# ilya16/deephumor

Measured on AMD Instinct MI355X. Metric: captions/sec (224x224, 32-tok, beam=5), higher is better.
Workload: dtype bf16; 1 GPU; C2 CaptioningLSTM + ImageEncoder (emb 256, hidden 512, 2 layers); images_per_gpu=256, global_batch=256, vocab=36541, max_len=32, beam_size=5, top_k=50, parallelism=image-sharded x1, one all_gather of token ids per batch, weights=synthetic name-keyed (seed 1234), inputs=device-resident fp32 NCHW images (host-inclusive rates under host_inclusive), hipgraph=False, schedule=sequential: one batch at a time

## Files before the change

deephumor_amd/csrc/beam.hip:

```cpp
#include "common.h"
#include "prof.h"

#define CAP DH_BEAM_MAX_SURVIVORS

__device__ __forceinline__ uint32_t f2key(float f) {
    uint32_t u = __float_as_uint(f);
    if (u == 0x80000000u) u = 0u;
    return (u & 0x80000000u) ? ~u : (u | 0x80000000u);
}


__device__ __forceinline__ void radix_pick_digit(const int* hist, int n_hist, int shift, uint32_t prefix,
                                                 uint32_t* s_prefix, int* s_k, int* wtot) {
    const int tid = threadIdx.x, lane = tid & 63, wave = tid >> 6;
    const int k = *s_k;
    int c = 0, suf = 0;
    if (tid < 256) {
        for (int h = 0; h < n_hist; ++h) c += hist[h * 256 + tid];
        suf = c;
        suf += __builtin_amdgcn_update_dpp(0, suf, 0x101, 0xF, 0xF, true);
        suf += __builtin_amdgcn_update_dpp(0, suf, 0x102, 0xF, 0xF, true);
        suf += __builtin_amdgcn_update_dpp(0, suf, 0x104, 0xF, 0xF, true);
        suf += __builtin_amdgcn_update_dpp(0, suf, 0x108, 0xF, 0xF, true);
        {
// ... 726 lines not shown
#pragma unroll
            for (int k = 0; k < MB; ++k) if (k == b) { was = was_ended[k] != 0; vb = val_b[k]; if constexpr (LN) kb = key_b[k]; }
            const int tok = was ? 0 : (pre ? L.pki[b * B + j] : p.pick_idx[(size_t)(base + b) * B + j]);
            ctok[c] = tok;
            cval[c] = vb + (was ? 0.f : (pre ? L.pkv[b * B + j] : p.pick_val[(size_t)(base + b) * B + j]));
            if constexpr (LN) q[c] = was ? kb : cval[c] * w_len;
            cpar[c] = b;
            cend[c] = (uint8_t)(was || tok == p.eos);
        }
        if (lane == 0) s_n = total;
    }
    wave_lds_sync();
    const int n = s_n;
    if constexpr (PL) {
        beam_pool_tail<MB>(p, img, lane, L, n, first, pre);
        return;
    }
    if constexpr (GR) {
        beam_group_tail(p, lane, L, n, first);
    } else if constexpr (DT) {
        if (!first) {
            for (int j = lane; j < B; j += 64) keep[j] = min(j, n - 1);
            wave_lds_sync();
            const float* rank = LN ? q : cval;
            for (int c = lane; c < n; c += 64) {
                const float me = rank[c];
                int r = 0;
                for (int j = 0; j < n; ++j) r += (rank[j] > me) || (rank[j] == me && j < c);
                if (r < B) keep[r] = c;
            }
        }
    } else if (!first) {
        float m = -INFINITY;
        for (int c = lane; c < n; c += 64) m = fmaxf(m, cval[c] / p.temperature);
        m = wave_max(m);
        float s = 0.f;
        for (int c = lane; c < n; c += 64) { const float e = expf(cval[c] / p.temperature - m); q[c] = e; s += e; }
        s = wave_sum(s);
        for (int c = lane; c < n; c += 64) {
            const float nz = p.noise ? p.noise[(size_t)img * B * B + c]
                                     : philox_exp1(p.seed ^ (p.seed_ptr ? *p.seed_ptr : 0ull), (uint32_t)(p.img0 + img), (uint32_t)p.step_index, 1u, 0u, (uint32_t)c);
            q[c] = (q[c] / s) / nz;
        }
        for (int j = lane; j < B; j += 64) keep[j] = min(j, n - 1);
        wave_lds_sync();
        for (int c = lane; c < n; c += 64) {
            const float me = q[c];
            int r = 0;
            for (int j = 0; j < n; ++j) r += (q[j] > me) || (q[j] == me && j < c);
            if (r < B) keep[r] = c;
        }
    }
    int32_t* tokbuf = stage;
    int32_t* srcbuf = stage + (size_t)B * p.tok_ld;
    if (!pre) {
        for (int i = lane; i < B * p.tok_ld; i += 64) tokbuf[i] = p.tokens[(size_t)base * p.tok_ld + i];
        if (p.src)
            for (int b = 0; b < B; ++b)
                for (int j = lane; j < p.t; j += 64) srcbuf[b * p.t + j] = p.src[(size_t)(base + b) * p.src_ld + j];
    }
    wave_lds_sync();
    int all_ended = 1;
    for (int b = 0; b < B; ++b) {
        const int c = keep[b], par = cpar[c];
        for (int i = lane; i < p.tok_ld; i += 64)
            p.tokens[(size_t)(base + b) * p.tok_ld + i] = (i == p.write_pos) ? ctok[c] : tokbuf[par * p.tok_ld + i];
        if (p.src) {
            for (int j = lane; j < p.t; j += 64) p.src[(size_t)(base + b) * p.src_ld + j] = srcbuf[par * p.t + j];
            if (lane == 0) p.src[(size_t)(base + b) * p.src_ld + p.t] = base + par;
        }
        if (lane == 0) {
            p.vals[base + b] = cval[c];
            if constexpr (LN) p.keys[base + b] = q[c];
            p.ended[base + b] = cend[c];
            p.parent[base + b] = base + par;
            p.hparent[base + b] = DT ? base + par : base + c / B;
        }
        all_ended &= cend[c];
    }
    if (lane == 0 && all_ended && !first) { p.done[img] = 1; p.end_step[img] = p.step_index; }
#undef s_n
}

template <int NT, bool PR, bool NU = false>
__global__ __launch_bounds__(NT) void beam_row_sample_groups_kernel(
    const float* __restrict__ logits, int ldl, int V, const float* __restrict__ gmax, int gm_ld, int n_groups,
    int gcols, int rows_per_img, int beam, int top_k, float temperature, int unk, const float* __restrict__ noise,
    uint64_t seed, const uint64_t* __restrict__ seed_ptr, int img0, int step, int32_t* __restrict__ pick_idx, float* __restrict__ pick_val,
    int32_t* __restrict__ err, const int32_t* __restrict__ first_pos, float top_p) {
    constexpr int MAXG = 1024, GPT = MAXG / NT;
    __shared__ int glist[MAXG];
    __shared__ int hist[4][256];
    __shared__ uint32_t s_prefix, s_thr;
    __shared__ int s_k, s_cnt, s_ng, wtot[4];
    __shared__ __attribute__((aligned(16))) int32_t pool[5 * CAP];
    int* const idx_a = pool; int* const idx_b = pool + CAP;
    float* const val_a = reinterpret_cast<float*>(pool + 2 * CAP); float* const val_b = reinterpret_cast<float*>(pool + 3 * CAP);
    float* const qv = reinterpret_cast<float*>(pool + 4 * CAP);
    __shared__ float red[NT];
    __shared__ int picks[DH_BEAM_MAX_BEAMS];
    const int rc = blockIdx.x, tid = threadIdx.x, lane = tid & 63, wave = tid >> 6;
    if constexpr (PR) { if (prompt_row_idle(first_pos, rc, rows_per_img, step)) return; }
    const float* row = logits + (size_t)rc * ldl;
    uint32_t gk[GPT];
#pragma unroll
    for (int e = 0; e < GPT; ++e) {
        const int g = tid + e * NT;
        const uint32_t k = f2key(gmax[(size_t)rc * gm_ld + min(g, n_groups - 1)]);
        gk[e] = g < n_groups ? k : 0u;
    }
    for (int i = tid; i < 512; i += NT) (&hist[0][0])[i] = 0;
    if (tid == 0) { s_prefix = 0u; s_k = min(top_k, n_groups); s_cnt = 0; s_ng = 0; s_thr = 0u; }
    __syncthreads();
#pragma unroll
    for (int pass = 0; pass < 2; ++pass) {
        const int shift = 24 - 8 * pass;
        const uint32_t prefix = s_prefix, mask = pass == 0 ? 0u : 0xFF000000u;
#pragma unroll
        for (int e = 0; e < GPT; ++e)
            if (tid + e * NT < n_groups && (gk[e] & mask) == prefix) atomicAdd(&hist[pass][(gk[e] >> shift) & 255u], 1);
        __syncthreads();
        radix_pick_digit(hist[pass], 1, shift, prefix, &s_prefix, &s_k, wtot);
    }
    const uint32_t bound = s_prefix;
#pragma unroll
    for (int e = 0; e < GPT; ++e)
        if (tid + e * NT < n_groups && gk[e] >= bound) glist[atomicAdd(&s_ng, 1)] = tid + e * NT;
    __syncthreads();
    const int ng = s_ng;
    constexpr int NWV = NT / 64, UN = 16;
    for (int q0 = wave; q0 < ng; q0 += NWV * UN) {
        float v[UN]; int ci[UN];
#pragma unroll
        for (int u = 0; u < UN; ++u) {
            const int q = q0 + u * NWV;
            ci[u] = q < ng ? glist[min(q, ng - 1)] * gcols + lane : V;
            v[u] = row[min(ci[u], V - 1)];
        }
#pragma unroll
        for (int u = 0; u < UN; ++u)
            if (lane < gcols && ci[u] < V && f2key(v[u]) >= bound) {
                const int pp = atomicAdd(&s_cnt, 1);
                if (pp < CAP) { idx_a[pp] = ci[u]; val_a[pp] = v[u]; }
            }
    }
    __syncthreads();
    if (s_cnt > CAP) radix_row_candidates<NT>(row, V, top_k, &hist[0][0], &s_prefix, &s_k, &s_cnt, wtot, idx_a, val_a);
    const RowLds L{idx_a, idx_b, val_a, val_b, qv, red, picks, &s_cnt, &s_thr};
    row_tail<NT, NU>(L, rc, ldl, rows_per_img, beam, top_k, temperature, unk, noise, seed, seed_ptr, img0, step, pick_idx, pick_val, err, top_p);
}

template <bool PR, bool NU = false>
static int row_sample_groups_launch(const float* logits, int ldl, int V, const float* group_max, int gm_ld,
                                    int n_groups, int group_cols, int rows, int rows_per_img, int beam,
                                    int top_k, float temperature, int unk_index, const float* noise,
                                    uint64_t seed, const uint64_t* seed_ptr, int img0, int step, const int32_t* first_pos,
                                    int32_t* pick_idx, float* pick_val, int32_t* err, void* stream, float top_p = 1.f) {
    DH_REQUIRE(logits && group_max && pick_idx && pick_val && err && rows > 0 && rows_per_img > 0 && V > 0 && ldl >= V);
    DH_REQUIRE(beam >= 1 && beam <= DH_BEAM_MAX_BEAMS && beam <= top_k && top_k <= V && temperature > 0.f);
    DH_REQUIRE(n_groups > 0 && n_groups <= 1024 && top_k <= n_groups && gm_ld >= n_groups && group_cols > 0 && group_cols <= 64 &&
               (long long)n_groups * group_cols >= V);
    DH_REQUIRE(!PR || (first_pos && rows_per_img == beam && rows % beam == 0));
    DhProfScope prof(NU ? "dh_beam_row_sample_nucleus" : "dh_beam_row_sample", 0.0, 0.0, stream);
    hipLaunchKernelGGL((beam_row_sample_groups_kernel<256, PR, NU>), dim3(rows), dim3(256), 0, (hipStream_t)stream, logits, ldl, V,
                       group_max, gm_ld, n_groups, group_cols, rows_per_img, beam, top_k, temperature, unk_index, noise,
                       seed, seed_ptr, img0, step, pick_idx, pick_val, err, first_pos, top_p);
    DH_LAUNCH_CHECK();
}

extern "C" int dh_beam_row_sample_groups(const float* logits, int ldl, int V, const float* group_max, int gm_ld,
                                         int n_groups, int group_cols, int rows, int rows_per_img, int beam,
                                         int top_k, float temperature, int unk_index, const float* noise,
                                         uint64_t seed, const uint64_t* __restrict__ seed_ptr, int img0, int step, int32_t* pick_idx, float* pick_val,
                                         int32_t* err, void* stream) {
    return row_sample_groups_launch<false>(logits, ldl, V, group_max, gm_ld, n_groups, group_cols, rows, rows_per_img, beam, top_k, temperature,
                                           unk_index, noise, seed, seed_ptr, img0, step, nullptr, pick_idx, pick_val, err, stream);
}

extern "C" int dh_beam_row_sample_groups_prompted(const float* logits, int ldl, int V, const float* group_max, int gm_ld,
                                                  int n_groups, int group_cols, int rows, int rows_per_img, int beam,
                                                  int top_k, float temperature, int unk_index, const float* noise,
                                                  uint64_t seed, const uint64_t* seed_ptr, int img0, int step, const int32_t* first_pos,
                                                  int32_t* pick_idx, float* pick_val, int32_t* err, void* stream) {
    return row_sample_groups_launch<true>(logits, ldl, V, group_max, gm_ld, n_groups, group_cols, rows, rows_per_img, beam, top_k, temperature,
                                          unk_index, noise, seed, seed_ptr, img0, step, first_pos, pick_idx, pick_val, err, stream);
}

template <bool PR, bool NU = false>
static int row_sample_launch(const float* logits, int ldl, int V, int rows, int rows_per_img, int beam,
                             int top_k, float temperature, int unk_index, const float* noise,
                             uint64_t seed, const uint64_t* seed_ptr, int img0, int step, const int32_t* first_pos, int32_t* pick_idx,
                             float* pick_val, int32_t* err, bool exact, void* stream, float top_p = 1.f) {
    DH_REQUIRE(logits && pick_idx && pick_val && err && rows > 0 && rows_per_img > 0 && V > 0 && ldl >= V);
    DH_REQUIRE(beam >= 1 && beam <= DH_BEAM_MAX_BEAMS && beam <= top_k && top_k <= V && temperature > 0.f);
    DH_REQUIRE(!PR || (first_pos && rows_per_img == beam && rows % beam == 0));
    DhProfScope prof(NU ? "dh_beam_row_sample_nucleus" : "dh_beam_row_sample", 0.0, 0.0, stream);
#define DH_FAST(EPT, NT, WPE) hipLaunchKernelGGL((beam_row_sample_fast_kernel<EPT, NT, WPE, PR, NU>), dim3(rows), dim3(NT), 0, \
        (hipStream_t)stream, logits, ldl, V, rows_per_img, beam, top_k, temperature, unk_index, noise, seed, seed_ptr, img0, \
        step, pick_idx, pick_val, err, first_pos, top_p)
    if (!exact && top_k <= 256 && V <= 512 * 8) DH_FAST(8, 512, 4);
    else if (!exact && top_k <= 256 && V <= 1024 * 16) DH_FAST(16, 1024, 8);
    else if (!exact && top_k <= 256 && V <= 1024 * 36) DH_FAST(36, 1024, 8);
    else if (!exact && top_k <= 256 && V <= 1024 * 64) DH_FAST(64, 1024, 4);
    else
        hipLaunchKernelGGL((beam_row_sample_kernel<PR, NU>), dim3(rows), dim3(256), 0, (hipStream_t)stream, logits, ldl, V,
                           rows_per_img, beam, top_k, temperature, unk_index, noise, seed, seed_ptr, img0, step, pick_idx,
                           pick_val, err, first_pos, top_p);
#undef DH_FAST
    DH_LAUNCH_CHECK();
}

extern "C" int dh_beam_row_sample(const float* logits, int ldl, int V, int rows, int rows_per_img, int beam,
                                  int top_k, float temperature, int unk_index, const float* noise,
                                  uint64_t seed, const uint64_t* __restrict__ seed_ptr, int img0, int step, int32_t* pick_idx, float* pick_val,
                                  int32_t* err, void* stream) {
    return row_sample_launch<false>(logits, ldl, V, rows, rows_per_img, beam, top_k, temperature, unk_index, noise, seed, seed_ptr, img0, step,
                                    nullptr, pick_idx, pick_val, err, false, stream);
}

extern "C" int dh_beam_row_sample_exact(const float* logits, int ldl, int V, int rows, int rows_per_img, int beam,
                                        int top_k, float temperature, int unk_index, const float* noise,
                                        uint64_t seed, const uint64_t* __restrict__ seed_ptr, int img0, int step, int32_t* pick_idx, float* pick_val,
                                        int32_t* err, void* stream) {
    return row_sample_launch<false>(logits, ldl, V, rows, rows_per_img, beam, top_k, temperature, unk_index, noise, seed, seed_ptr, img0, step,
                                    nullptr, pick_idx, pick_val, err, true, stream);
}

extern "C" int dh_beam_row_sample_prompted(const float* logits, int ldl, int V, int rows, int rows_per_img, int beam,
                                           int top_k, float temperature, int unk_index, const float* noise,
                                           uint64_t seed, const uint64_t* seed_ptr, int img0, int step, const int32_t* first_pos,
                                           int32_t* pick_idx, float* pick_val, int32_t* err, void* stream) {
    return row_sample_launch<true>(logits, ldl, V, rows, rows_per_img, beam, top_k, temperature, unk_index, noise, seed, seed_ptr, img0, step,
                                   first_pos, pick_idx, pick_val, err, false, stream);
}

extern "C" int dh_beam_row_sample_exact_prompted(const float* logits, int ldl, int V, int rows, int rows_per_img, int beam,
                                                 int top_k, float temperature, int unk_index, const float* noise,
                                                 uint64_t seed, const uint64_t* seed_ptr, int img0, int step, const int32_t* first_pos,
                                                 int32_t* pick_idx, float* pick_val, int32_t* err, void* stream) {
    return row_sample_launch<true>(logits, ldl, V, rows, rows_per_img, beam, top_k, temperature, unk_index, noise, seed, seed_ptr, img0, step,
                                   first_pos, pick_idx, pick_val, err, true, stream);
}

extern "C" int dh_beam_row_sample_nucleus(const float* logits, int ldl, int V, const float* group_max, int gm_ld, int n_groups,
                                          int group_cols, int rows, int rows_per_img, int beam, int top_k, float top_p,
                                          float temperature, int unk_index, const float* noise, uint64_t seed, const uint64_t* seed_ptr,
                                          int img0, int step, const int32_t* first_pos, int exact, int32_t* pick_idx, float* pick_val,
                                          int32_t* err, void* stream) {
    DH_REQUIRE(top_p > 0.f && top_p < 1.f);
// ... 418 lines not shown
    p.diversity = diversity_penalty;
    const size_t lds = (size_t)beam * (tok_ld + (src ? t : 0)) * sizeof(int32_t);
    DH_REQUIRE(lds <= 56 * 1024);
    const dim3 grid(n_img), block(64);
    if (first_pos) {
        if (beam <= 16) hipLaunchKernelGGL((beam_select_groups_kernel<16, true>), grid, block, lds, (hipStream_t)stream, p);
        else hipLaunchKernelGGL((beam_select_groups_kernel<DH_BEAM_MAX_BEAMS, true>), grid, block, lds, (hipStream_t)stream, p);
    } else {
        if (beam <= 16) hipLaunchKernelGGL((beam_select_groups_kernel<16, false>), grid, block, lds, (hipStream_t)stream, p);
        else hipLaunchKernelGGL((beam_select_groups_kernel<DH_BEAM_MAX_BEAMS, false>), grid, block, lds, (hipStream_t)stream, p);
    }
    DH_LAUNCH_CHECK();
}

__global__ __launch_bounds__(64) void beam_finalize_pool_kernel(
    const int32_t* __restrict__ tokens, int tok_ld, const float* __restrict__ keys, const uint8_t* __restrict__ ended,
    const uint8_t* __restrict__ done, const int32_t* __restrict__ pool_tokens, const float* __restrict__ pool_keys,
    const int32_t* __restrict__ pool_len, const int32_t* __restrict__ pool_n, int32_t* __restrict__ out_tokens, int out_ld,
    int32_t* __restrict__ out_len, float* __restrict__ out_score, int32_t* __restrict__ out_index, int32_t* __restrict__ out_drawn,
    int32_t* __restrict__ out_row_len, int beam, int full_len, int pad_index) {
    __shared__ int s_from[DH_BEAM_MAX_BEAMS], s_len[DH_BEAM_MAX_BEAMS];
    const int img = blockIdx.x, lane = threadIdx.x, B = beam, base = img * B;
    const int cap = min(out_ld, tok_ld);
    const int n_pool = min(max(pool_n[img], 0), B);
    const bool in_pool = lane < n_pool;
    const bool live = lane < B && !done[img] && !ended[base + lane];
    float pk = in_pool ? pool_keys[base + lane] : -INFINITY;
    float lk = live ? keys[base + lane] : -INFINITY;
    if (!(pk == pk)) pk = -INFINITY;
    if (!(lk == lk)) lk = -INFINITY;
    const int plen = in_pool ? min(max(pool_len[base + lane], 0), cap) : 0;
    const int llen = min(max(full_len, 0), cap);
    int prank = lane, lrank = 0;
    for (int j = 0; j < B; ++j) {
        const float opk = __shfl(pk, j), olk = __shfl(lk, j);
        const bool o_pool = j < n_pool, o_live = __shfl((int)live, j) != 0;
        prank += o_live && olk > pk;
        lrank += (o_pool && opk >= lk) + (o_live && (olk > lk || (olk == lk && j < lane)));
    }
    const int n_live = __popcll(__ballot(live));
    const int total = n_pool + n_live;
    const unsigned long long idle = __ballot(lane < B && !live);
    const int frank = total + __popcll(idle & ((1ull << lane) - 1ull));
    if (lane < B) { s_from[lane] = lane; s_len[lane] = 0; }
    __syncthreads();
    if (in_pool && prank < B) {
        s_from[prank] = -1 - lane; s_len[prank] = plen;
        out_score[base + prank] = pk; out_index[base + prank] = -1; out_len[base + prank] = plen;
    }
    if (live && lrank < B) {
        s_from[lrank] = lane; s_len[lrank] = llen;
        out_score[base + lrank] = lk; out_index[base + lrank] = lane; out_len[base + lrank] = llen;
    }
    if (lane < B && !live && frank < B) {
        s_from[frank] = lane; s_len[frank] = llen;
        out_score[base + frank] = -INFINITY; out_index[base + frank] = lane; out_len[base + frank] = llen;
    }
    __syncthreads();
    if (lane == 0) { out_drawn[img] = 0; out_row_len[img] = s_len[0]; }
    for (int s = 0; s < B; ++s) {
        const int from = s_from[s], len = s_len[s];
        const int32_t* __restrict__ row = from < 0 ? pool_tokens + (size_t)(base + (-1 - from)) * tok_ld : tokens + (size_t)(base + from) * tok_ld;
        int32_t* __restrict__ dst = out_tokens + (size_t)(base + s) * out_ld;
        for (int i = lane; i < out_ld; i += 64) dst[i] = i < len ? row[i] : pad_index;
    }
}

extern "C" int dh_beam_finalize_pool(const int32_t* tokens, int tok_ld, const float* keys, const uint8_t* ended, const uint8_t* done,
                                     const int32_t* pool_tokens, const float* pool_keys, const int32_t* pool_len, const int32_t* pool_n,
                                     int32_t* out_tokens, int out_ld, int32_t* out_len, float* out_score, int32_t* out_index,
                                     int32_t* out_drawn, int32_t* out_row_len, int n_img, int beam, int full_len, int pad_index,
                                     void* stream) {
    DH_REQUIRE(tokens && keys && ended && done && pool_tokens && pool_keys && pool_len && pool_n);
    DH_REQUIRE(out_tokens && out_len && out_score && out_index && out_drawn && out_row_len);
    DH_REQUIRE(n_img > 0 && tok_ld > 0 && out_ld > 0 && full_len >= 0 && beam >= 1 && beam <= DH_BEAM_MAX_BEAMS);
    DhProfScope prof("dh_beam_finalize_pool", 0.0, 0.0, stream);
    hipLaunchKernelGGL(beam_finalize_pool_kernel, dim3(n_img), dim3(64), 0, (hipStream_t)stream, tokens, tok_ld, keys, ended, done,
                       pool_tokens, pool_keys, pool_len, pool_n, out_tokens, out_ld, out_len, out_score, out_index, out_drawn, out_row_len,
                       beam, full_len, pad_index);
    DH_LAUNCH_CHECK();
}


__device__ __forceinline__ float key2f(uint32_t k) {
    return __uint_as_float((k & 0x80000000u) ? (k & 0x7FFFFFFFu) : ~k);
}

__global__ __launch_bounds__(256) void beam_filter_topk_kernel(float* __restrict__ logits, int ldl, int V, int top_k, int unk) {
    __shared__ int hist[4 * 256];
    __shared__ uint32_t s_prefix;
    __shared__ int s_k, wtot[4];
    const int tid = threadIdx.x, hw = tid >> 6;
    float* row = logits + (size_t)blockIdx.x * ldl;
    if (tid == 0) { s_prefix = 0u; s_k = top_k; }
    uint32_t mask = 0u;
    for (int pass = 0; pass < 4; ++pass) {
        const int shift = 24 - 8 * pass;
        for (int i = tid; i < 1024; i += 256) hist[i] = 0;
        __syncthreads();
        const uint32_t prefix = s_prefix;
        for (int i = tid; i < V; i += 256) {
            const uint32_t key = f2key(row[i]);
            if ((key & mask) == prefix) atomicAdd(&hist[hw * 256 + ((key >> shift) & 255u)], 1);
        }
        __syncthreads();
        radix_pick_digit(hist, 4, shift, prefix, &s_prefix, &s_k, wtot);
        mask |= 0xFFu << shift;
    }
    const float thr = key2f(s_prefix);
    for (int i = tid; i < V; i += 256)
        if (row[i] < thr || i == unk) row[i] = -INFINITY;
}

__global__ __launch_bounds__(256) void beam_sample_k_kernel(const float* __restrict__ x, int ld, int V, int k, float temperature,
                                                            const float* __restrict__ noise, int noise_ld, uint64_t seed,
                                                            const uint64_t* __restrict__ seed_ptr, int stream_id, int draw,
                                                            int64_t* __restrict__ out, int32_t* __restrict__ err) {
    __shared__ float red[256];
    __shared__ float rq[256];
    __shared__ int ri[256];
    __shared__ int picked[64];
    const int tid = threadIdx.x, r = blockIdx.x;
    const float* row = x + (size_t)r * ld;
    float m = -INFINITY;
    for (int i = tid; i < V; i += 256) m = fmaxf(m, row[i] / temperature);
    m = block_reduce_256(m, red, true);
    if (m == -INFINITY) {
        if (tid == 0) atomicOr(err, DH_BEAM_ERR_ALL_FILTERED);
        for (int j = tid; j < k; j += 256) out[(size_t)r * k + j] = 0;
        return;
    }
    float s = 0.f, cnt = 0.f;
    for (int i = tid; i < V; i += 256) { const float e = expf(row[i] / temperature - m); s += e; cnt += e > 0.f ? 1.f : 0.f; }
    s = block_reduce_256(s, red, false);
    cnt = block_reduce_256(cnt, red, false);
    if (tid == 0 && cnt < (float)k) atomicOr(err, DH_BEAM_ERR_TOO_FEW);
    const uint64_t sd = seed ^ (seed_ptr ? *seed_ptr : 0ull);
    for (int round = 0; round < k; ++round) {
        float bq = -1.f; int bi = 0x7FFFFFFF;
        for (int i = tid; i < V; i += 256) {
            bool taken = false;
            for (int j = 0; j < round; ++j) taken |= picked[j] == i;
            if (taken) continue;
            const float nz = noise ? noise[(size_t)r * noise_ld + i] : philox_exp1(sd, (uint32_t)stream_id, (uint32_t)draw, 3u, (uint32_t)r, (uint32_t)i);
            const float q = (expf(row[i] / temperature - m) / s) / nz;
            if (q > bq) { bq = q; bi = i; }
        }
        rq[tid] = bq; ri[tid] = bi;
        __syncthreads();
        for (int st = 128; st > 0; st >>= 1) {
            if (tid < st) {
                const float oq = rq[tid + st]; const int oi = ri[tid + st];
                if (oq > rq[tid] || (oq == rq[tid] && oi < ri[tid])) { rq[tid] = oq; ri[tid] = oi; }
            }
            __syncthreads();
        }
        if (tid == 0) { picked[round] = ri[0]; out[(size_t)r * k + round] = ri[0] == 0x7FFFFFFF ? 0 : ri[0]; }
        __syncthreads();
    }
}

__global__ void beam_gather_kernel(const float* __restrict__ values, int ld, int V, const int64_t* __restrict__ indices, int k,
                                   float* __restrict__ out, int total, int32_t* __restrict__ err) {
    const int t = blockIdx.x * blockDim.x + threadIdx.x;
    if (t >= total) return;
    const int64_t i = indices[t];
    if (i < 0 || i >= V) { if (err) atomicOr(err, DH_BEAM_ERR_OVERFLOW); out[t] = 0.f; return; }
    out[t] = values[(size_t)(t / k) * ld + i];
}

// ... 200 lines not shown
```

deephumor_amd/csrc/lstm_wreg.hip:

```cpp
#include "common.h"
#include "prof.h"

__device__ uint4 lw_zero_page[4];

namespace {
struct LstmWregParams {
    const uint16_t* x_rows; int ldx, x_div;
    const uint16_t* emb; const int32_t* tokens; int tok_ld, tok_pos;
    const uint16_t* h_prev; const float* c_prev; const int32_t* hparent;
    uint16_t* h_next; float* c_next;
    uint16_t* h_out; int ld_out;
    const uint4* wp; const float* bias;
    int rows, row_mult, E, Hh, tiles_m, tiles_n;
};

__device__ __forceinline__ float lw_sigmoid(float x) { return __frcp_rn(1.0f + __expf(-x)); }
__device__ __forceinline__ float lw_tanh(float x) {
    const float e = __expf(-2.0f * fabsf(x));
    const float t = (1.0f - e) * __frcp_rn(1.0f + e);
    return copysignf(t, x);
}

__device__ __forceinline__ void lw_dma16(const void* base, unsigned off, void* lds_dst) {
    const unsigned m = __builtin_amdgcn_readfirstlane((unsigned)(uintptr_t)(dh_lptr_t)lds_dst);
    asm volatile("s_mov_b32 m0, %0\n\ts_nop 0\n\tglobal_load_lds_dwordx4 %1, %2" :: "s"(m), "v"(off), "s"(base) : "memory");
}

template <typename OT, int NSLAB>
__global__ __launch_bounds__(512, 1) void lstm_wreg_kernel(LstmWregParams p) {
    constexpr int BM = 80, TM = 5, RG = BM / 8, KF = 2 * NSLAB, SLABB = BM * 128, PF = 3;
    __shared__ __attribute__((aligned(16))) unsigned char lds[NSLAB * SLABB];
    const int tid = threadIdx.x, lane = tid & 63;
    const int wave = __builtin_amdgcn_readfirstlane(tid >> 6);
    const int l15 = lane & 15, lq = lane >> 4, lr = lane >> 3, lpos = lane & 7;
    int cb, rb;
    if ((p.tiles_n & 7) == 0) {
        const int xcd = blockIdx.x & 7, idx = blockIdx.x >> 3;
        cb = xcd * (p.tiles_n >> 3) + idx / p.tiles_m; rb = idx % p.tiles_m;
    } else {
        cb = blockIdx.x % p.tiles_n; rb = blockIdx.x / p.tiles_n;
    }
    const int m0 = rb * BM, n0 = cb * 128;
    const int N = 4 * p.Hh;

    unsigned xo[RG], ho[RG];
#pragma unroll
    for (int g = 0; g < RG; ++g) {
        const int m = min(m0 + g * 8 + lr, p.rows - 1);
        const int rl = m * p.row_mult;
        xo[g] = p.tokens ? (unsigned)p.tokens[(size_t)rl * p.tok_ld + p.tok_pos] * (unsigned)p.E : (unsigned)(m / p.x_div) * (unsigned)p.ldx;
        ho[g] = (unsigned)(p.hparent ? p.hparent[rl] : rl) * (unsigned)p.Hh;
    }
    int hp_e[TM];
#pragma unroll
    for (int i = 0; i < TM; ++i) {
        const int m = min(m0 + 16 * i + l15, p.rows - 1);
        hp_e[i] = p.hparent ? p.hparent[m * p.row_mult] : m * p.row_mult;
    }
    const int u = (n0 + 16 * wave) / 4 + lq;
    const float4 b4 = *reinterpret_cast<const float4*>(p.bias + n0 + 16 * wave + 4 * lq);
    float c0[TM];
#pragma unroll
    for (int i = 0; i < TM; ++i) c0[i] = p.c_prev ? p.c_prev[(size_t)hp_e[i] * p.Hh + u] : 0.f;
    {
        const uint16_t* xbase = p.tokens ? p.emb : p.x_rows;
        const unsigned swz8 = (unsigned)((lpos ^ lr) << 3);
#pragma unroll
        for (int sl = 0; sl < (NSLAB + 7) / 8; ++sl) {
            const int s = wave + 8 * sl;
            if (s < NSLAB) {
                const int k = 64 * s;
                unsigned char* dst = lds + s * SLABB;
                if (k < p.E) {
#pragma unroll
                    for (int g = 0; g < RG; ++g) lw_dma16(xbase, (xo[g] + k + swz8) * 2u, dst + g * 1024);
                } else if (p.h_prev) {
#pragma unroll
                    for (int g = 0; g < RG; ++g) lw_dma16(p.h_prev, (ho[g] + (k - p.E) + swz8) * 2u, dst + g * 1024);
                } else {
#pragma unroll
                    for (int g = 0; g < RG; ++g) dh_lds_dma16(lw_zero_page, dst + g * 1024);
                }
            }
        }
    }
    uint4 wf[KF];
    {
        const uint4* wsrc = p.wp + ((size_t)(n0 / 16 + wave)) * 64 + lane;
        const size_t fstep = (size_t)(N / 16) * 64;
#pragma unroll
        for (int f = 0; f < KF; ++f) wf[f] = wsrc[(size_t)f * fstep];
    }
    asm volatile("s_waitcnt vmcnt(0)" ::: "memory");
    __syncthreads();

    dh_f32x4 acc[TM];
#pragma unroll
    for (int i = 0; i < TM; ++i) acc[i] = dh_f32x4{0.f, 0.f, 0.f, 0.f};
    unsigned rd_base[2][3];
#pragma unroll
    for (int kk = 0; kk < 2; ++kk)
#pragma unroll
        for (int wdw = 0; wdw < 3; ++wdw) {
            rd_base[kk][wdw] = (unsigned)(l15 * 128 + (((kk * 4 + lq) ^ (l15 & 7)) << 4) + wdw * 61440);
            asm volatile("" : "+v"(rd_base[kk][wdw]));
        }
    uint4 fa[PF + 1];
    auto rd = [&](int t) {
        const int f = t / TM, i = t - f * TM, s = f >> 1, kk = f & 1;
        const int off = s * SLABB + i * 2048, wdw = off / 61440;
        fa[t % (PF + 1)] = *reinterpret_cast<const uint4*>(lds + rd_base[kk][wdw] + (off - wdw * 61440));
    };
#pragma unroll
    for (int t = 0; t < PF; ++t) rd(t);
#pragma unroll
    for (int t = 0; t < KF * TM; ++t) {
        const int f = t / TM, i = t - f * TM;
        if (t + PF < KF * TM) rd(t + PF);
        acc[i] = Op16<OT>::mfma(wf[f], fa[t % (PF + 1)], acc[i]);
        __builtin_amdgcn_sched_barrier(0);
    }
#pragma unroll
    for (int i = 0; i < TM; ++i) {
        const int m = m0 + 16 * i + l15;
        if (m >= p.rows) continue;
        const size_t rl = (size_t)m * p.row_mult;
        const float gi = acc[i][0] + b4.x, gf = acc[i][1] + b4.y, gg = acc[i][2] + b4.z, go = acc[i][3] + b4.w;
        const float c1 = lw_sigmoid(gf) * c0[i] + lw_sigmoid(gi) * lw_tanh(gg);
        const float h1 = lw_sigmoid(go) * lw_tanh(c1);
        const uint16_t hb = Op16<OT>::from_f32(h1);
        p.c_next[rl * p.Hh + u] = c1;
        p.h_next[rl * p.Hh + u] = hb;
        p.h_out[(size_t)m * p.ld_out + u] = hb;
    }
}
}

extern "C" int dh_lstm_layer_wreg_supported(int E, int Hh) {
    const int K = E + Hh;
    return (E % 64) == 0 && (Hh % 32) == 0 && (K == 768 || K == 1024);
}

extern "C" int dh_lstm_layer_wreg(const void* x_rows, int ldx, int x_div, const void* emb, const int32_t* tokens, int tok_ld,
                                  int tok_pos, const void* h_prev, const float* c_prev, const int32_t* hparent, void* h_next,
                                  float* c_next, void* h_out, int ld_out, const void* w_packed, const float* b_il, int rows,
                                  int row_mult, int E, int Hh, int dtype, void* stream) {
    if (!DH_IS_16BIT(dtype)) return DH_ERR_UNSUPPORTED;
    DH_REQUIRE((x_rows || (emb && tokens)) && h_next && c_next && h_out && w_packed && b_il && dh_lstm_layer_wreg_supported(E, Hh));
    DH_REQUIRE(rows > 0 && row_mult > 0 && x_div > 0 && (ldx % 8) == 0 && ld_out >= Hh);
    DH_REQUIRE((h_prev == nullptr) == (c_prev == nullptr) && h_prev != h_next && c_prev != c_next);
    DH_REQUIRE(((uintptr_t)w_packed % 16) == 0 && ((uintptr_t)b_il % 16) == 0 && ((uintptr_t)x_rows % 16) == 0 &&
               ((uintptr_t)emb % 16) == 0 && ((uintptr_t)h_prev % 16) == 0);
    LstmWregParams p{};
    p.x_rows = (const uint16_t*)x_rows; p.ldx = ldx; p.x_div = x_div;
    p.emb = (const uint16_t*)emb; p.tokens = tokens; p.tok_ld = tok_ld; p.tok_pos = tok_pos;
    p.h_prev = (const uint16_t*)h_prev; p.c_prev = c_prev; p.hparent = hparent;
    p.h_next = (uint16_t*)h_next; p.c_next = c_next; p.h_out = (uint16_t*)h_out; p.ld_out = ld_out;
    p.wp = (const uint4*)w_packed; p.bias = b_il; p.rows = rows; p.row_mult = row_mult; p.E = E; p.Hh = Hh;
    p.tiles_m = dh_cdiv(rows, 80); p.tiles_n = (4 * Hh) / 128;
    const double K = E + Hh;
    DhProfScope prof("dh_lstm_layer_fused", 2.0 * rows * 4 * Hh * K, 2.0 * (rows * K + 4.0 * Hh * K) + 12.0 * rows * Hh, stream);
    const dim3 grid(p.tiles_m * p.tiles_n);
    hipStream_t s = (hipStream_t)stream;
    DH_DISPATCH_16(dtype, {
        if (E + Hh == 768) hipLaunchKernelGGL((lstm_wreg_kernel<T, 12>), grid, dim3(512), 0, s, p);
        else hipLaunchKernelGGL((lstm_wreg_kernel<T, 16>), grid, dim3(512), 0, s, p);
    });
    DH_LAUNCH_CHECK();
}
```

Before: 36570 captions/s.

## Rewrite grouped row top-k sampling kernel as single-wavefront with ballot-based selection

Replaces the 256-thread row sampling kernel, which used LDS radix histograms and block barriers, with a 64-thread single-wave kernel. Group and candidate thresholds are found by bitwise ballot/popcount bisection, and compaction uses mbcnt prefixes instead of LDS atomics. Candidate columns are gathered through buffer loads batched 64 at a time, and the tail (softmax, noise, beam picks) runs wave-locally. The aim is to cut barrier and atomic overhead on this small per-row kernel. In exchange each row gets fewer threads and more register pressure from the 64-element load batch.

```diff
diff --git a/deephumor_amd/csrc/beam.hip b/deephumor_amd/csrc/beam.hip
--- a/deephumor_amd/csrc/beam.hip
+++ b/deephumor_amd/csrc/beam.hip
@@ -832,72 +832,278 @@
 #undef s_n
 }
 
-template <int NT, bool PR, bool NU = false>
-__global__ __launch_bounds__(NT) void beam_row_sample_groups_kernel(
+
+__device__ __forceinline__ int wave_prefix(uint64_t mask) {
+    return (int)__builtin_amdgcn_mbcnt_hi((uint32_t)(mask >> 32), __builtin_amdgcn_mbcnt_lo((uint32_t)mask, 0u));
+}
+
+__device__ __forceinline__ int wave_excl_scan_i(int v, int lane, int* total) {
+    int inc = v;
+    inc += __builtin_amdgcn_update_dpp(0, inc, 0x111, 0xF, 0xF, true);
+    inc += __builtin_amdgcn_update_dpp(0, inc, 0x112, 0xF, 0xF, true);
+    inc += __builtin_amdgcn_update_dpp(0, inc, 0x114, 0xF, 0xF, true);
+    inc += __builtin_amdgcn_update_dpp(0, inc, 0x118, 0xF, 0xF, true);
+    const int t0 = __builtin_amdgcn_readlane(inc, 15), t1 = __builtin_amdgcn_readlane(inc, 31), t2 = __builtin_amdgcn_readlane(inc, 47),
+              t3 = __builtin_amdgcn_readlane(inc, 63);
+    const int drow = lane >> 4;
+    *total = t0 + t1 + t2 + t3;
+    return inc - v + (drow == 0 ? 0 : drow == 1 ? t0 : drow == 2 ? t0 + t1 : t0 + t1 + t2);
+}
+
+__device__ __forceinline__ float key2f(uint32_t key) {
+    return __uint_as_float((key & 0x80000000u) ? (key & 0x7FFFFFFFu) : ~key);
+}
+
+template <typename T, typename F>
+__device__ __forceinline__ void wave_for_each(const T* buf, int n, int lane, F&& f) {
+    for (int j0 = 0; j0 < n; j0 += 64) {
+        const int x = __builtin_bit_cast(int, buf[min(j0 + lane, n - 1)]);
+        const int cnt = min(64, n - j0);
+#pragma unroll 4
+        for (int jj = 0; jj < cnt; ++jj) f(__builtin_bit_cast(T, __builtin_amdgcn_readlane(x, jj)), j0 + jj);
+    }
+}
+
+template <bool NU>
+__device__ __forceinline__ void row_tail_wave(const RowLds& L, int n_cand, int lane, int rc, int ldl, int rows_per_img, int beam, int top_k,
+                                              float temperature, int unk, const float* __restrict__ noise, uint64_t seed,
+                                              const uint64_t* __restrict__ seed_ptr, int img0, int step, int32_t* __restrict__ pick_idx,
+                                              float* __restrict__ pick_val, int32_t* __restrict__ err, float top_p) {
+    int* const cidx = L.idx_a; float* const cval = L.val_a; int* const idx = L.idx_b; float* const val = L.val_b;
+    float* const pv = L.val_a; int* const ord = L.idx_a;
+    float* qv = L.qv; int* picks = L.picks;
+    int n0 = n_cand;
+    if (n0 > CAP) { if (lane == 0) atomicOr(err, DH_BEAM_ERR_OVERFLOW); n0 = CAP; }
+    const uint32_t key0 = lane < n0 ? f2key(cval[lane]) : 0u;
+    uint32_t thr = 0u;
+#pragma unroll 1
+    for (uint32_t bit = 0x80000000u; bit != 0u; bit >>= 1) {
+        const uint32_t probe = thr | bit;
+        int c = __builtin_popcountll(__builtin_amdgcn_ballot_w64(key0 >= probe));
+        for (int i = 64 + lane; i - lane < n0; i += 64)
+            c += __builtin_popcountll(__builtin_amdgcn_ballot_w64(i < n0 && f2key(cval[min(i, n0 - 1)]) >= probe));
+        if (c >= top_k) thr = probe;
+    }
+    int n = 0;
+    for (int i0 = 0; i0 < n0; i0 += 64) {
+        const int i = i0 + lane, ic = min(i, n0 - 1);
+        const float v = cval[ic];
+        const int id = cidx[ic];
+        const bool keep = i < n0 && f2key(v) >= thr && id != unk;
+        const uint64_t mask = __builtin_amdgcn_ballot_w64(keep);
+        if (keep) { const int p = n + wave_prefix(mask); idx[p] = id; val[p] = v; }
+        n += __builtin_popcountll(mask);
+    }
+    wave_lds_sync();
+    if (n == 0) {
+        if (lane == 0) atomicOr(err, DH_BEAM_ERR_ALL_FILTERED);
+        if (lane < beam) pick_store(pick_idx, pick_val, (size_t)rc * beam + lane, 0, 0.f);
+        return;
+    }
+    float m = -INFINITY;
+    for (int i = lane; i < n; i += 64) m = fmaxf(m, val[i] / temperature);
+    m = wave_max(m);
+    float s = 0.f;
+    for (int w = 0; w < 4 && w * 64 < n; ++w) {
+        float part = 0.f;
+        for (int i = w * 64 + lane; i < n; i += 256) { const float e = expf(val[i] / temperature - m); qv[i] = e; part += e; }
+        part = wave_sum(part);
+        s = w == 0 ? part : s + part;
+    }
+    if (dh_softmax_nonfinite(m, s)) {
+        if (lane == 0) atomicOr(err, DH_BEAM_ERR_NONFINITE);
+        if (lane < beam) pick_store(pick_idx, pick_val, (size_t)rc * beam + lane, 0, 0.f);
+        return;
+    }
+    const int img = rc / rows_per_img, rin = rc % rows_per_img;
+    for (int i = lane; i < n; i += 64) {
+        const float nz = noise ? noise[(size_t)rc * ldl + idx[i]]
+                               : philox_exp1(seed ^ (seed_ptr ? *seed_ptr : 0ull), (uint32_t)(img0 + img), (uint32_t)step, 0u, (uint32_t)rin, (uint32_t)idx[i]);
+        if constexpr (NU) pv[i] = qv[i] / s;
+        qv[i] = (qv[i] / s) / nz;
+    }
+    wave_lds_sync();
+    if constexpr (NU) {
+        for (int i0 = 0; i0 < n; i0 += 64) {
+            const int i = i0 + lane;
+            const float me = pv[min(i, n - 1)];
+            int r = 0;
+            wave_for_each(pv, n, lane, [&](float o, int j) { r += (o > me) || (o == me && j < i); });
+            if (i < n) ord[r] = i;
+        }
+        wave_lds_sync();
+        constexpr int IPT = CAP / 256;
+        float below = 0.f;
+        for (int w = 0; w < 4 && w * 64 * IPT < n; ++w) {
+            const int t = w * 64 + lane;
+            float loc[IPT], run = 0.f;
+#pragma unroll
+            for (int k = 0; k < IPT; ++k) {
+                const int pos = t * IPT + k;
+                loc[k] = pos < n ? pv[ord[min(pos, n - 1)]] : 0.f;
+                run += loc[k];
+            }
+            float inc = run;
+            inc += dpp_shr0<0x111>(inc); inc += dpp_shr0<0x112>(inc); inc += dpp_shr0<0x114>(inc); inc += dpp_shr0<0x118>(inc);
+            const float t0 = lane_get(inc, 15), t1 = lane_get(inc, 31), t2 = lane_get(inc, 47), t3 = lane_get(inc, 63);
+            const int drow = lane >> 4;
+            float pre = (drow == 0 ? 0.f : drow == 1 ? t0 : drow == 2 ? t0 + t1 : (t0 + t1) + t2) + dpp_shr0<0x111>(inc);
+            pre += below;
+#pragma unroll
+            for (int k = 0; k < IPT; ++k) {
+                const int pos = t * IPT + k;
+                if (pos < n && !(pre < top_p || pos < beam)) qv[ord[pos]] = -1.f;
+                pre += loc[k];
+            }
+            below += ((t0 + t1) + t2) + t3;
+        }
+        wave_lds_sync();
+    }
+    int pi = -1;
+    const float q0 = qv[min(lane, n - 1)];
+    if (n <= 64 && beam <= 8 && __builtin_amdgcn_ballot_w64(lane < n && q0 != q0) == 0ull) {
+        bool open = lane < n;
+        for (int b = 0; b < beam; ++b) {
+            const float best = wave_max(open ? q0 : -INFINITY);
+            const uint64_t at = __builtin_amdgcn_ballot_w64(open && q0 == best);
+            if (at == 0ull) break;
+            const int w = __builtin_ctzll(at);
+            if (lane == b) pi = w;
+            if (lane == w) open = false;
+        }
+    } else {
+        picks[lane] = -1;
+        static_assert(DH_BEAM_MAX_BEAMS == 64, "one pick slot per lane");
+        wave_lds_sync();
+        for (int i0 = 0; i0 < n; i0 += 64) {
+            const int i = i0 + lane;
+            const float me = qv[min(i, n - 1)];
+            int r = 0;
+            wave_for_each(qv, n, lane, [&](float o, int j) { r += (o > me) || (o == me && j < i); });
+            if (i < n && r < beam) picks[r] = i;
+        }
+        wave_lds_sync();
+        pi = lane < beam ? picks[lane] : -1;
+    }
+    if (lane == 0 && n < beam) atomicOr(err, DH_BEAM_ERR_TOO_FEW);
+    const float lv = pi >= 0 ? val[pi] : -INFINITY;
+    const float mx = wave_max(lv);
+    const float se = wave_sum(pi >= 0 ? expf(lv - mx) : 0.f);
+    const float lse = logf(se);
+    if (lane < beam) pick_store(pick_idx, pick_val, (size_t)rc * beam + lane, pi >= 0 ? idx[pi] : 0, pi >= 0 ? (lv - mx) - lse : -INFINITY);
+}
+
+template <int GPT, bool PR, bool NU = false>
+__global__ __launch_bounds__(64) void beam_row_sample_groups_kernel(
     const float* __restrict__ logits, int ldl, int V, const float* __restrict__ gmax, int gm_ld, int n_groups,
     int gcols, int rows_per_img, int beam, int top_k, float temperature, int unk, const float* __restrict__ noise,
     uint64_t seed, const uint64_t* __restrict__ seed_ptr, int img0, int step, int32_t* __restrict__ pick_idx, float* __restrict__ pick_val,
     int32_t* __restrict__ err, const int32_t* __restrict__ first_pos, float top_p) {
-    constexpr int MAXG = 1024, GPT = MAXG / NT;
-    __shared__ int glist[MAXG];
-    __shared__ int hist[4][256];
-    __shared__ uint32_t s_prefix, s_thr;
-    __shared__ int s_k, s_cnt, s_ng, wtot[4];
     __shared__ __attribute__((aligned(16))) int32_t pool[5 * CAP];
     int* const idx_a = pool; int* const idx_b = pool + CAP;
     float* const val_a = reinterpret_cast<float*>(pool + 2 * CAP); float* const val_b = reinterpret_cast<float*>(pool + 3 * CAP);
     float* const qv = reinterpret_cast<float*>(pool + 4 * CAP);
-    __shared__ float red[NT];
+    int* const glist = idx_b;
     __shared__ int picks[DH_BEAM_MAX_BEAMS];
-    const int rc = blockIdx.x, tid = threadIdx.x, lane = tid & 63, wave = tid >> 6;
+    const int rc = blockIdx.x, lane = threadIdx.x;
     if constexpr (PR) { if (prompt_row_idle(first_pos, rc, rows_per_img, step)) return; }
     const float* row = logits + (size_t)rc * ldl;
     uint32_t gk[GPT];
 #pragma unroll
     for (int e = 0; e < GPT; ++e) {
-        const int g = tid + e * NT;
+        const int g = lane + e * 64;
         const uint32_t k = f2key(gmax[(size_t)rc * gm_ld + min(g, n_groups - 1)]);
         gk[e] = g < n_groups ? k : 0u;
     }
-    for (int i = tid; i < 512; i += NT) (&hist[0][0])[i] = 0;
-    if (tid == 0) { s_prefix = 0u; s_k = min(top_k, n_groups); s_cnt = 0; s_ng = 0; s_thr = 0u; }
-    __syncthreads();
-#pragma unroll
-    for (int pass = 0; pass < 2; ++pass) {
-        const int shift = 24 - 8 * pass;
-        const uint32_t prefix = s_prefix, mask = pass == 0 ? 0u : 0xFF000000u;
-#pragma unroll
-        for (int e = 0; e < GPT; ++e)
-            if (tid + e * NT < n_groups && (gk[e] & mask) == prefix) atomicAdd(&hist[pass][(gk[e] >> shift) & 255u], 1);
-        __syncthreads();
-        radix_pick_digit(hist[pass], 1, shift, prefix, &s_prefix, &s_k, wtot);
-    }
-    const uint32_t bound = s_prefix;
-#pragma unroll
-    for (int e = 0; e < GPT; ++e)
-        if (tid + e * NT < n_groups && gk[e] >= bound) glist[atomicAdd(&s_ng, 1)] = tid + e * NT;
-    __syncthreads();
-    const int ng = s_ng;
-    constexpr int NWV = NT / 64, UN = 16;
-    for (int q0 = wave; q0 < ng; q0 += NWV * UN) {
-        float v[UN]; int ci[UN];
-#pragma unroll
-        for (int u = 0; u < UN; ++u) {
-            const int q = q0 + u * NWV;
-            ci[u] = q < ng ? glist[min(q, ng - 1)] * gcols + lane : V;
-            v[u] = row[min(ci[u], V - 1)];
-        }
-#pragma unroll
-        for (int u = 0; u < UN; ++u)
-            if (lane < gcols && ci[u] < V && f2key(v[u]) >= bound) {
-                const int pp = atomicAdd(&s_cnt, 1);
-                if (pp < CAP) { idx_a[pp] = ci[u]; val_a[pp] = v[u]; }
+    const int kk = min(top_k, n_groups);
+    uint32_t bound = 0u;
+#pragma unroll 1
+    for (uint32_t bit = 0x80000000u; bit >= 0x10000u; bit >>= 1) {
+        const uint32_t probe = bound | bit;
+        int c = 0;
+#pragma unroll
+        for (int e = 0; e < GPT; ++e) c += __builtin_popcountll(__builtin_amdgcn_ballot_w64(gk[e] >= probe));
+        if (c >= kk) bound = probe;
+    }
+    int ng = 0;
+#pragma unroll
+    for (int e = 0; e < GPT; ++e) {
+        const int g = lane + e * 64;
+        const bool sel = g < n_groups && gk[e] >= bound;
+        const uint64_t mask = __builtin_amdgcn_ballot_w64(sel);
+        if (sel) glist[ng + wave_prefix(mask)] = g;
+        ng += __builtin_popcountll(mask);
+    }
+    wave_lds_sync();
+    const float bound_f = key2f(bound);
+    const __amdgpu_buffer_rsrc_t rsrc = __builtin_amdgcn_make_buffer_rsrc(const_cast<float*>(row), 0, V * 4, 0x00020000);
+    int cnt = 0;
+    for (int q0 = 0; q0 < ng; q0 += 64) {
+        const int gl = glist[min(q0 + lane, ng - 1)];
+        float v[64];
+#pragma unroll
+        for (int u = 0; u < 64; ++u)
+            v[u] = __builtin_bit_cast(float, __builtin_amdgcn_raw_buffer_load_b32(rsrc, lane * 4, __builtin_amdgcn_readlane(gl, u) * gcols * 4, 0));
+        __builtin_amdgcn_sched_barrier(0);
+        int mlo = 0, mhi = 0;
+#pragma unroll
+        for (int u = 0; u < 64; ++u) {
+            const uint64_t at = __builtin_amdgcn_ballot_w64(!(v[u] < bound_f));
+            mlo = lane == u ? (int)(uint32_t)at : mlo;
+            mhi = lane == u ? (int)(uint32_t)(at >> 32) : mhi;
+        }
+        const int c0 = gl * gcols;
+        const int ncol = q0 + lane < ng ? max(0, min(gcols, V - c0)) : 0;
+        uint64_t mask = ((uint64_t)(uint32_t)mhi << 32) | (uint32_t)mlo;
+        mask &= ncol >= 64 ? ~0ull : (1ull << ncol) - 1ull;
+        int total;
+        int p = cnt + wave_excl_scan_i(__builtin_popcountll(mask), lane, &total);
+        if (cnt + total <= CAP) {
+            while (__builtin_amdgcn_ballot_w64(mask != 0ull) != 0ull) {
+                const bool on1 = mask != 0ull;
+                const int j1 = __builtin_ctzll(mask | (1ull << 63));
+                mask &= mask - 1ull;
+                const bool on2 = mask != 0ull;
+                const int j2 = __builtin_ctzll(mask | (1ull << 63));
+                mask &= mask - 1ull;
+                const float x1 = row[min(c0 + j1, V - 1)], x2 = row[min(c0 + j2, V - 1)];
+                if (on1) { idx_a[p] = c0 + j1; val_a[p] = x1; }
+                if (on2) { idx_a[p + 1] = c0 + j2; val_a[p + 1] = x2; }
+                p += (int)on1 + (int)on2;
             }
-    }
-    __syncthreads();
-    if (s_cnt > CAP) radix_row_candidates<NT>(row, V, top_k, &hist[0][0], &s_prefix, &s_k, &s_cnt, wtot, idx_a, val_a);
-    const RowLds L{idx_a, idx_b, val_a, val_b, qv, red, picks, &s_cnt, &s_thr};
-    row_tail<NT, NU>(L, rc, ldl, rows_per_img, beam, top_k, temperature, unk, noise, seed, seed_ptr, img0, step, pick_idx, pick_val, err, top_p);
+        }
+        cnt += total;
+    }
+    if (cnt > CAP) {
+        uint32_t thr = 0u;
+#pragma unroll 1
+        for (uint32_t bit = 0x80000000u; bit != 0u; bit >>= 1) {
+            const uint32_t probe = thr | bit;
+            int c = 0;
+#pragma unroll 4
+            for (int q = 0; q < ng; ++q) {
+                const int ci = glist[q] * gcols + lane;
+                const float x = row[min(ci, V - 1)];
+                c += __builtin_popcountll(__builtin_amdgcn_ballot_w64(lane < gcols && ci < V && f2key(x) >= probe));
+            }
+            if (c >= top_k) thr = probe;
+        }
+        cnt = 0;
+#pragma unroll 4
+        for (int q = 0; q < ng; ++q) {
+            const int ci = glist[q] * gcols + lane;
+            const float x = row[min(ci, V - 1)];
+            const bool cand = lane < gcols && ci < V && f2key(x) >= thr;
+            const uint64_t mask = __builtin_amdgcn_ballot_w64(cand);
+            const int pp = cnt + wave_prefix(mask);
+            if (cand && pp < CAP) { idx_a[pp] = ci; val_a[pp] = x; }
+            cnt += __builtin_popcountll(mask);
+        }
+    }
+    wave_lds_sync();
+    const RowLds L{idx_a, idx_b, val_a, val_b, qv, nullptr, picks, nullptr, nullptr};
+    row_tail_wave<NU>(L, cnt, lane, rc, ldl, rows_per_img, beam, top_k, temperature, unk, noise, seed, seed_ptr, img0, step, pick_idx, pick_val,
+                      err, top_p);
 }
 
 template <bool PR, bool NU = false>
@@ -912,9 +1118,13 @@
                (long long)n_groups * group_cols >= V);
     DH_REQUIRE(!PR || (first_pos && rows_per_img == beam && rows % beam == 0));
     DhProfScope prof(NU ? "dh_beam_row_sample_nucleus" : "dh_beam_row_sample", 0.0, 0.0, stream);
-    hipLaunchKernelGGL((beam_row_sample_groups_kernel<256, PR, NU>), dim3(rows), dim3(256), 0, (hipStream_t)stream, logits, ldl, V,
-                       group_max, gm_ld, n_groups, group_cols, rows_per_img, beam, top_k, temperature, unk_index, noise,
-                       seed, seed_ptr, img0, step, pick_idx, pick_val, err, first_pos, top_p);
+#define DH_GROUPS(GPT) hipLaunchKernelGGL((beam_row_sample_groups_kernel<GPT, PR, NU>), dim3(rows), dim3(64), 0, (hipStream_t)stream, \
+        logits, ldl, V, group_max, gm_ld, n_groups, group_cols, rows_per_img, beam, top_k, temperature, unk_index, noise, seed, seed_ptr, \
+        img0, step, pick_idx, pick_val, err, first_pos, top_p)
+    if (n_groups <= 4 * 64) DH_GROUPS(4);
+    else if (n_groups <= 10 * 64) DH_GROUPS(10);
+    else DH_GROUPS(16);
+#undef DH_GROUPS
     DH_LAUNCH_CHECK();
 }
 
@@ -1499,10 +1709,6 @@
 }
 
 
-__device__ __forceinline__ float key2f(uint32_t k) {
-    return __uint_as_float((k & 0x80000000u) ? (k & 0x7FFFFFFFu) : ~k);
-}
-
 __global__ __launch_bounds__(256) void beam_filter_topk_kernel(float* __restrict__ logits, int ldl, int V, int top_k, int unk) {
     __shared__ int hist[4 * 256];
     __shared__ uint32_t s_prefix;
```

New measurement: 36740 captions/s, median of 5. Within noise of the previous version (+0.5%).

## Stage LSTM cell outputs through LDS for coalesced 16-byte stores; hoist weight loads

Applied to the files above, without the earlier changes.

The epilogue now writes c and h results into a swizzled LDS tile and then issues coalesced 16-byte global stores for c_next, h_next and h_out. Before, each lane did scattered 4-byte and 2-byte stores. The weight-register loads are also issued earlier, ahead of the activation DMA, and the index gathers are split by branch, so more global latency can overlap. The cost is an extra LDS round trip and a barrier. For the 16-slab case the output tile reuses the slab region after a sync, and the host now requires 16-byte alignment on the outputs.

```diff
diff --git a/deephumor_amd/csrc/lstm_wreg.hip b/deephumor_amd/csrc/lstm_wreg.hip
--- a/deephumor_amd/csrc/lstm_wreg.hip
+++ b/deephumor_amd/csrc/lstm_wreg.hip
@@ -29,7 +29,8 @@
 template <typename OT, int NSLAB>
 __global__ __launch_bounds__(512, 1) void lstm_wreg_kernel(LstmWregParams p) {
     constexpr int BM = 80, TM = 5, RG = BM / 8, KF = 2 * NSLAB, SLABB = BM * 128, PF = 3;
-    __shared__ __attribute__((aligned(16))) unsigned char lds[NSLAB * SLABB];
+    constexpr int TILEB = BM * (128 + 64);
+    __shared__ __attribute__((aligned(16))) unsigned char lds[NSLAB * SLABB + TILEB <= 163840 ? NSLAB * SLABB + TILEB : NSLAB * SLABB];
     const int tid = threadIdx.x, lane = tid & 63;
     const int wave = __builtin_amdgcn_readfirstlane(tid >> 6);
     const int l15 = lane & 15, lq = lane >> 4, lr = lane >> 3, lpos = lane & 7;
@@ -43,27 +44,52 @@
     const int m0 = rb * BM, n0 = cb * 128;
     const int N = 4 * p.Hh;
 
-    unsigned xo[RG], ho[RG];
-#pragma unroll
-    for (int g = 0; g < RG; ++g) {
-        const int m = min(m0 + g * 8 + lr, p.rows - 1);
-        const int rl = m * p.row_mult;
-        xo[g] = p.tokens ? (unsigned)p.tokens[(size_t)rl * p.tok_ld + p.tok_pos] * (unsigned)p.E : (unsigned)(m / p.x_div) * (unsigned)p.ldx;
-        ho[g] = (unsigned)(p.hparent ? p.hparent[rl] : rl) * (unsigned)p.Hh;
-    }
+    unsigned xi[RG], hi[RG];
     int hp_e[TM];
-#pragma unroll
-    for (int i = 0; i < TM; ++i) {
-        const int m = min(m0 + 16 * i + l15, p.rows - 1);
-        hp_e[i] = p.hparent ? p.hparent[m * p.row_mult] : m * p.row_mult;
-    }
+    auto lrow = [&](int g) { return min(m0 + g * 8 + lr, p.rows - 1); };
+    auto erow = [&](int i) { return min(m0 + 16 * i + l15, p.rows - 1); };
+    if (p.tokens) {
+#pragma unroll
+        for (int g = 0; g < RG; ++g) xi[g] = (unsigned)p.tokens[(size_t)(lrow(g) * p.row_mult) * p.tok_ld + p.tok_pos];
+    } else {
+#pragma unroll
+        for (int g = 0; g < RG; ++g) xi[g] = (unsigned)(lrow(g) / p.x_div);
+    }
+    if (p.hparent) {
+#pragma unroll
+        for (int g = 0; g < RG; ++g) hi[g] = (unsigned)p.hparent[lrow(g) * p.row_mult];
+#pragma unroll
+        for (int i = 0; i < TM; ++i) hp_e[i] = p.hparent[erow(i) * p.row_mult];
+    } else {
+#pragma unroll
+        for (int g = 0; g < RG; ++g) hi[g] = (unsigned)(lrow(g) * p.row_mult);
+#pragma unroll
+        for (int i = 0; i < TM; ++i) hp_e[i] = erow(i) * p.row_mult;
+    }
+    asm volatile("" ::: "memory");
     const int u = (n0 + 16 * wave) / 4 + lq;
+    uint4 wf[KF];
+    {
+        const uint4* wsrc = p.wp + ((size_t)(n0 / 16 + wave)) * 64 + lane;
+        const size_t fstep = (size_t)(N / 16) * 64;
+#pragma unroll
+        for (int f = 0; f < KF; ++f) wf[f] = wsrc[(size_t)f * fstep];
+    }
     const float4 b4 = *reinterpret_cast<const float4*>(p.bias + n0 + 16 * wave + 4 * lq);
+#pragma unroll
+    for (int g = 0; g < RG; ++g) asm volatile("" : "+v"(xi[g]), "+v"(hi[g]) :: "memory");
+#pragma unroll
+    for (int i = 0; i < TM; ++i) asm volatile("" : "+v"(hp_e[i]) :: "memory");
     float c0[TM];
 #pragma unroll
-    for (int i = 0; i < TM; ++i) c0[i] = p.c_prev ? p.c_prev[(size_t)hp_e[i] * p.Hh + u] : 0.f;
+    for (int i = 0; i < TM; ++i) c0[i] = 0.f;
+    if (p.c_prev) {
+#pragma unroll
+        for (int i = 0; i < TM; ++i) c0[i] = p.c_prev[(size_t)hp_e[i] * p.Hh + u];
+    }
     {
         const uint16_t* xbase = p.tokens ? p.emb : p.x_rows;
+        const unsigned xmul = (unsigned)(p.tokens ? p.E : p.ldx);
         const unsigned swz8 = (unsigned)((lpos ^ lr) << 3);
 #pragma unroll
         for (int sl = 0; sl < (NSLAB + 7) / 8; ++sl) {
@@ -73,23 +99,16 @@
                 unsigned char* dst = lds + s * SLABB;
                 if (k < p.E) {
 #pragma unroll
-                    for (int g = 0; g < RG; ++g) lw_dma16(xbase, (xo[g] + k + swz8) * 2u, dst + g * 1024);
+                    for (int g = 0; g < RG; ++g) lw_dma16(xbase, (xi[g] * xmul + k + swz8) * 2u, dst + g * 1024);
                 } else if (p.h_prev) {
 #pragma unroll
-                    for (int g = 0; g < RG; ++g) lw_dma16(p.h_prev, (ho[g] + (k - p.E) + swz8) * 2u, dst + g * 1024);
+                    for (int g = 0; g < RG; ++g) lw_dma16(p.h_prev, (hi[g] * (unsigned)p.Hh + (k - p.E) + swz8) * 2u, dst + g * 1024);
                 } else {
 #pragma unroll
                     for (int g = 0; g < RG; ++g) dh_lds_dma16(lw_zero_page, dst + g * 1024);
                 }
             }
         }
-    }
-    uint4 wf[KF];
-    {
-        const uint4* wsrc = p.wp + ((size_t)(n0 / 16 + wave)) * 64 + lane;
-        const size_t fstep = (size_t)(N / 16) * 64;
-#pragma unroll
-        for (int f = 0; f < KF; ++f) wf[f] = wsrc[(size_t)f * fstep];
     }
     asm volatile("s_waitcnt vmcnt(0)" ::: "memory");
     __syncthreads();
@@ -120,18 +139,35 @@
         acc[i] = Op16<OT>::mfma(wf[f], fa[t % (PF + 1)], acc[i]);
         __builtin_amdgcn_sched_barrier(0);
     }
+    unsigned char* ct = lds + (NSLAB * SLABB + TILEB <= 163840 ? NSLAB * SLABB : 0);
+    unsigned char* ht = ct + BM * 128;
+    if constexpr (NSLAB * SLABB + TILEB > 163840) __syncthreads();
 #pragma unroll
     for (int i = 0; i < TM; ++i) {
-        const int m = m0 + 16 * i + l15;
-        if (m >= p.rows) continue;
-        const size_t rl = (size_t)m * p.row_mult;
+        const int r = 16 * i + l15;
         const float gi = acc[i][0] + b4.x, gf = acc[i][1] + b4.y, gg = acc[i][2] + b4.z, go = acc[i][3] + b4.w;
         const float c1 = lw_sigmoid(gf) * c0[i] + lw_sigmoid(gi) * lw_tanh(gg);
         const float h1 = lw_sigmoid(go) * lw_tanh(c1);
-        const uint16_t hb = Op16<OT>::from_f32(h1);
-        p.c_next[rl * p.Hh + u] = c1;
-        p.h_next[rl * p.Hh + u] = hb;
-        p.h_out[(size_t)m * p.ld_out + u] = hb;
+        *reinterpret_cast<float*>(ct + r * 128 + ((wave ^ (l15 & 7)) << 4) + lq * 4) = c1;
+        *reinterpret_cast<uint16_t*>(ht + r * 64 + (((wave >> 1) ^ ((l15 >> 1) & 3)) << 4) + ((wave & 1) * 4 + lq) * 2) =
+            Op16<OT>::from_f32(h1);
+    }
+    __syncthreads();
+    const int ub = n0 / 4;
+#pragma unroll
+    for (int id = tid; id < BM * 8; id += 512) {
+        const int r = id >> 3, ch = id & 7, m = m0 + r;
+        if (m < p.rows)
+            *reinterpret_cast<uint4*>(p.c_next + (size_t)m * p.row_mult * p.Hh + ub + 4 * ch) =
+                *reinterpret_cast<const uint4*>(ct + r * 128 + ((ch ^ (r & 7)) << 4));
+    }
+    if (tid >= 512 - BM * 4) {
+        const int id = tid - (512 - BM * 4), r = id >> 2, hc = id & 3, m = m0 + r;
+        if (m < p.rows) {
+            const uint4 v = *reinterpret_cast<const uint4*>(ht + r * 64 + ((hc ^ ((r >> 1) & 3)) << 4));
+            *reinterpret_cast<uint4*>(p.h_next + (size_t)m * p.row_mult * p.Hh + ub + 8 * hc) = v;
+            *reinterpret_cast<uint4*>(p.h_out + (size_t)m * p.ld_out + ub + 8 * hc) = v;
+        }
     }
 }
 }
@@ -151,6 +187,7 @@
     DH_REQUIRE((h_prev == nullptr) == (c_prev == nullptr) && h_prev != h_next && c_prev != c_next);
     DH_REQUIRE(((uintptr_t)w_packed % 16) == 0 && ((uintptr_t)b_il % 16) == 0 && ((uintptr_t)x_rows % 16) == 0 &&
                ((uintptr_t)emb % 16) == 0 && ((uintptr_t)h_prev % 16) == 0);
+    DH_REQUIRE(((uintptr_t)h_next % 16) == 0 && ((uintptr_t)c_next % 16) == 0 && ((uintptr_t)h_out % 16) == 0 && (ld_out % 8) == 0);
     LstmWregParams p{};
     p.x_rows = (const uint16_t*)x_rows; p.ldx = ldx; p.x_div = x_div;
     p.emb = (const uint16_t*)emb; p.tokens = tokens; p.tok_ld = tok_ld; p.tok_pos = tok_pos;
```

Result: faster. 35880 captions/s before, 36710 captions/s after (median of 6 runs) (+2.3%).
